# LJacksonPan/RaTrack

Hardware: AMD Instinct MI355X
Metric: radar frame-pairs/sec (backbone forward, eval) at B=64,N=256 per GPU (higher is better)
Workload: dtype f32 (2xfp16 split MFMA: three fp16 products per fp32 product, fp32 accumulate, power-of-two scales per matrix and position); 1 GPU; Track4D.backbone forward, B=64 frame-pairs x N=256 points per GPU, S=512 centroids, eval-mode BN, random-init weights, hipGraph=True, batches in flight=4; global_batch=64, parallelism=replicas x1 (no collective on the forward path)

## Files before the change

include/rtk_fused.h:

```cpp
#ifndef RTK_FUSED_H
#define RTK_FUSED_H

#include "rtk_pointnet2.h"

#ifdef __cplusplus
extern "C" {
#endif

#define RTK_MAX_SRC 4
#define RTK_MAX_LAYERS 4

typedef struct {
    const float *ptr;
    int pitch;
    int channels;
    int per_sample;
} rtk_src_t;

#define RTK_LAYER_SPLIT 0x100
typedef struct {
    const float *w_packed;
    const float *bias;
    int cin16, cout16;
    int act;
// ... 78 lines not shown
RTK_EXPORT int rtk_sa_scale_split(int samples, int n, int npoint, int nsample, const float *xyz, const float *new_xyz,
                                  const int *idx, const float *q, int q_pitch, int c1, const float *w1xyz_packed,
                                  const void *split_image, const float *image_scale, const float *bias2, float *out, int out_pitch,
                                  int out_offset, const int *src_nuniq, const int *dst_nuniq, rtk_stream_t stream);
RTK_EXPORT int rtk_sa_scale_split_serial(int samples, int n, int npoint, int nsample, const float *xyz, const float *new_xyz,
                                         const int *idx, const float *q, int q_pitch, int c1, const float *w1xyz_packed,
                                         const void *split_image, const float *image_scale, const float *bias2, float *out,
                                         int out_pitch, int out_offset, const int *src_nuniq, const int *dst_nuniq,
                                         rtk_stream_t stream);
RTK_EXPORT int rtk_split_mlp2(int positions, const float *x, const void *images, const float *image_scales, const float *bias1,
                              const float *bias2, float *y, rtk_stream_t stream);

RTK_EXPORT int rtk_prepare_inputs(int b, int n, const float *pc1, const float *pc2, const float *feature1,
                                  const float *feature2, float *xyz, float *raw, rtk_stream_t stream);

RTK_EXPORT int rtk_fps_centroids(int b, int n, int npoint, const float *xyz, int *idx, float *new_xyz, int *nuniq,
                                 int *tie, const int *n_valid, float *snap, int *first_tie, rtk_stream_t stream);

RTK_EXPORT int rtk_knn_point_masked(int b, int s, int n, int k, const float *query, const float *points, int64_t *idx,
                                    const int *n_valid, rtk_stream_t stream);

RTK_EXPORT int rtk_fps_relevel(int b, int npoint, int levels, const float *xyz1, const int *nuniq1, const int *tie,
                               int *idx, float *new_xyz, int *nuniq, int *tie_work, const int *idx1, const float *snap1,
                               int snap_pitch, const int *first_tie1, rtk_stream_t stream);

RTK_EXPORT int rtk_gru_step(int b, int layers, int hidden, const float *x, const float *h_in, const float *w_ih,
                            const float *w_hh, const float *b_ih, const float *b_hh, float *h_out, float *y,
                            rtk_stream_t stream);

RTK_EXPORT int rtk_gru_step_head(int b, int layers, int hidden, const float *x, const float *h_in, const float *w_ih,
                                 const float *w_hh, const float *b_ih, const float *b_hh, float *h_out, float *y, const float *head_wt,
                                 const float *head_bias, float *head_out, int head_cout, rtk_stream_t stream);

#define RTK_GT_MAX_JOBS 4
typedef struct {
    const float *wt, *bias;
    float *out;
    int cout, s0, count, out_pitch;
    const float *wt2;
    int s2;
} rtk_gterm_job_t;
RTK_EXPORT int rtk_global_terms(int samples, int cin, const float *g, int njobs, const rtk_gterm_job_t *jobs, float *bcast, int bcast_pitch,
                                int n, rtk_stream_t stream);

#define RTK_COPY_MAX_JOBS 8
typedef struct {
    const void *src;
    void *dst;
    long bytes;
} rtk_copy_job_t;
RTK_EXPORT int rtk_copy_multi(int njobs, const rtk_copy_job_t *jobs, rtk_stream_t stream);

RTK_EXPORT int rtk_to_channel_major(int samples, int n, int channels, const float *src, int src_pitch, int per_sample,
                                    float *dst, int dst_channels, int dst_channel_offset, rtk_stream_t stream);

RTK_EXPORT int rtk_ball_query_pair(int b, int n, int npoint, float radius1, int nsample1, float radius2, int nsample2,
                                   const float *new_xyz, const float *xyz, int *idx1, int *idx2, const int *nuniq,
                                   rtk_stream_t stream);

RTK_EXPORT int rtk_three_nn_masked(int b, int n, int m, const float *unknown, const float *known, float *dist2, int *idx,
                                   const int *unknown_nuniq, const int *known_nuniq, rtk_stream_t stream);

RTK_EXPORT int rtk_geometry_front(int b, int clouds, int n, int npoint, const float *frame1, const float *frame2, int channel_major,
                                  const float *feature1, const float *feature2, float *xyz, float *raw, int *fps_idx, float *new_xyz,
                                  int *nuniq, int *tie, int *first_tie, float *snap, const int *n_valid, int64_t *knn12, int64_t *knn11,
                                  const float *q1_w, float *q1_out, int q1_cout, rtk_stream_t stream);
// ... 72 lines not shown
```

ratrack_amd/abi.py:

```python
import ctypes

import torch

_i, _l, _f, _d, _p = ctypes.c_int, ctypes.c_long, ctypes.c_float, ctypes.c_double, ctypes.c_void_p
_ip, _fp, _pp, P = ctypes.POINTER(_i), ctypes.POINTER(_f), ctypes.POINTER(_p), ctypes.POINTER



class Src(ctypes.Structure):
    _fields_ = [("ptr", _p), ("pitch", _i), ("channels", _i), ("per_sample", _i)]


class Layer(ctypes.Structure):
    _fields_ = [("w_packed", _p), ("bias", _p), ("cin16", _i), ("cout16", _i), ("act", _i), ("inv_scale", _f)]


class Interp(ctypes.Structure):
    _fields_ = [("known_feats", _p), ("pitch", _i), ("channels", _i), ("m", _i), ("idx", _p), ("dist2", _p), ("nuniq", _p)]


class GtermJob(ctypes.Structure):
    _fields_ = [("wt", _p), ("bias", _p), ("out", _p), ("cout", _i), ("s0", _i), ("count", _i), ("out_pitch", _i), ("wt2", _p), ("s2", _i)]


# ... 121 lines not shown
    "rtk_group_points": [_i] * 5 + [_p] * 3 + [_p],
    "rtk_group_points_grad": [_i] * 5 + [_p] * 3 + [_p],
    "rtk_group_points_grad_set": [_i] * 5 + [_p] * 3 + [_p],
    "rtk_three_nn": [_i] * 3 + [_p] * 4 + [_p],
    "rtk_knn": [_i] * 4 + [_p] * 4 + [_p],
    "rtk_three_interpolate": [_i] * 4 + [_p] * 4 + [_p],
    "rtk_three_interpolate_grad": [_i] * 4 + [_p] * 4 + [_p],
    "rtk_three_interpolate_grad_set": [_i] * 4 + [_p] * 4 + [_p],
    "rtk_knn_point": [_i] * 4 + [_p] * 3 + [_p],
    "rtk_pointwise_mlp": [_i, _i, P(Interp), _i, P(Src), _p, _i, P(Layer), _p, _i, _i, _i, _p, _p, _p],
    "rtk_pointwise_mlp_pipelined": [_i, _i, P(Interp), _i, P(Src), _p, _i, P(Layer), _p, _i, _i, _i, _p, _p, _p],
    "rtk_pointwise_mlp_tap": [_i, _i, P(Interp), P(Layer), _p, _i, _p, P(Layer), _i, _p, _i, _p],
    "rtk_pointwise_mlp_tap_pipelined": [_i, _i, P(Interp), P(Layer), _p, _i, _p, P(Layer), _i, _p, _i, _p],
    "rtk_pointwise_mlp_pair": [_i, _i, _i, P(Src), _p, P(Layer), _p, _i, _i, _i, P(Layer), _p, _i, _p],
    "rtk_sa_scale": [_i] * 4 + [_p] * 4 + [_i, _i, _p, _i, P(Layer), _p, _i, _i, _p, _p, _p],
    "rtk_sa_scale_serial": [_i] * 4 + [_p] * 4 + [_i, _i, _p, _i, P(Layer), _p, _i, _i, _p, _p, _p],
    "rtk_cost_volume": [_i] * 3 + [_p] * 6 + [P(Layer), P(Layer), _p, _i, _p],
    "rtk_patch_cost": [_i] * 2 + [_p] * 3 + [_i, P(Layer), _p, _i, _i, _p],
    "rtk_patch_cost_wave16": [_i] * 2 + [_p] * 3 + [_i, P(Layer), _p, _i, _i, _p],
    "rtk_pack_split_layer": [_i, _i, _p, _i, _p, _p, _p],
    "rtk_cost_volume_split": [_i] * 3 + [_p] * 10 + [P(Layer), _p, _i, _p],
    "rtk_cost_volume_split_shared": [_i] * 3 + [_p] * 10 + [P(Layer), _p, _i, _i, _p],
    "rtk_cost_volume_split_gconst": [_i] * 3 + [_p] * 10 + [P(Layer), _p, _i, _i, _p],
    "rtk_cost_volume_split_term": [_i] * 3 + [_p] * 11 + [P(Layer), _p, _i, _i, _p],
    "rtk_sa_scale_split": [_i] * 4 + [_p] * 4 + [_i, _i, _p, _p, _p, _p, _p, _i, _i, _p, _p, _p],
    "rtk_sa_scale_split_serial": [_i] * 4 + [_p] * 4 + [_i, _i, _p, _p, _p, _p, _p, _i, _i, _p, _p, _p],
    "rtk_split_mlp2": [_i, _p, _p, _p, _p, _p, _p, _p],
    "rtk_prepare_inputs": [_i] * 2 + [_p] * 6 + [_p],
    "rtk_fps_centroids": [_i] * 3 + [_p] * 8 + [_p],
    "rtk_knn_point_masked": [_i] * 4 + [_p] * 4 + [_p],
    "rtk_fps_relevel": [_i] * 3 + [_p] * 9 + [_i, _p, _p],
    "rtk_gru_step": [_i] * 3 + [_p] * 8 + [_p],
    "rtk_gru_step_head": [_i] * 3 + [_p] * 11 + [_i, _p],
    "rtk_global_terms": [_i, _i, _p, _i, P(GtermJob), _p, _i, _i, _p],
    "rtk_copy_multi": [_i, P(CopyJob), _p],
    "rtk_to_channel_major": [_i] * 3 + [_p, _i, _i, _p, _i, _i, _p],
    "rtk_ball_query_pair": [_i] * 3 + [_f, _i, _f, _i] + [_p] * 5 + [_p],
    "rtk_three_nn_masked": [_i] * 3 + [_p] * 6 + [_p],
    "rtk_geometry_front": [_i] * 4 + [_p, _p, _i] + [_p] * 13 + [_p, _p, _i, _p],
    "rtk_geometry_tables": [_i] * 3 + [_p] * 3 + [_fp, _ip, _pp, _pp, _pp, _p],
    "rtk_to_channel_major_multi": [_i] * 3 + [_p, _p],
    "rtk_log_sinkhorn": [_i, _i, _p, _f, _i, _p, _p],
    "rtk_dbscan": [_i, _p, _i, _p, _p, _f, _d, _i, _p, _p],
    "rtk_dbscan_batched": [_p, _f, _d, _i, _i, _p, _p, _p, _p, _p, _l, _p],
    "rtk_object_descriptors": [_p, _i, _p, _p, _p, _p, _p, _p],
    "rtk_affinity_pairs": [_i, _i] + [_p] * 7 + [_p],
    "rtk_associate_batched": [_i] * 3 + [_p] * 7 + [_f, _i] + [_p] * 9 + [_p],
    "rtk_associate_optimal": [_i] * 3 + [_p] * 7 + [_d] + [_p] * 9 + [_p],
    "rtk_associate_optimal_lds_bytes": [_i],
    "rtk_track_memory": [_i] * 3 + [_p] * 21 + [_p],
    "rtk_track_memory_motion": [_i] * 3 + [_f] + [_p] * 24 + [_p],
    "rtk_track_max_objects": [],
    "rtk_gt_labels": [_p, _p, _p],
    "rtk_eval_frame": [_p, _p, _p, _p],
    "rtk_gt_objects_lds_bytes": [_i, _i],
    "rtk_track_score_lds_bytes": [_i, _i, _i],
    "rtk_track_score_memory_lds_bytes": [_i, _i, _i],
    "rtk_gt_objects": [_p, _p, _p],
    "rtk_track_score": [_p, _p, _p, _p],
    "rtk_track_score_logged": [_p, _p, _p, _p, _p],
    "rtk_track_score_memory": [_p, _p, _p, _p, _p, _p],
    "rtk_score_track_means": [_i, _p, _p, _p, _p],
    "rtk_score_thresholds": [_p, _p, _p, _i, _p, _p, _p],
    "rtk_score_replay": [_i, _i, _p, _p, _p, _p, _i, _p, _p, _p, _p],
    "rtk_score_hota": [_i, _i, _p, _p, _p, _i, _p, _p, _p, _p],
    "rtk_score_identity_lds_bytes": [_i],
# ... 69 lines not shown
```

ratrack_amd/csrc/fused_misc.hip:

```cpp
#include <math.h>

#include "assoc_common.h"
#include "rtk_common.h"
#include "rtk_fused.h"
#include "rtk_train.h"

__global__ void prepare_inputs_kernel(int b, int n, const float *__restrict__ pc1, const float *__restrict__ pc2,
                                      const float *__restrict__ f1, const float *__restrict__ f2, float *__restrict__ xyz,
                                      float *__restrict__ raw) {
    const long t = (long)blockIdx.x * blockDim.x + threadIdx.x;
    if (t >= 2L * b * n) return;
    const int s = (int)(t / n), p = (int)(t % n);
    const bool second = s >= b;
    const int sb = second ? s - b : s;
    const float *pc = second ? pc2 : pc1;
    const float *f = second ? f2 : f1;
    xyz[t * 3 + 0] = pc[((long)sb * 3 + 0) * n + p];
    xyz[t * 3 + 1] = pc[((long)sb * 3 + 1) * n + p];
    xyz[t * 3 + 2] = pc[((long)sb * 3 + 2) * n + p];
    *reinterpret_cast<float4 *>(raw + t * 4) = make_float4(f[((long)sb * 2 + 0) * n + p], f[((long)sb * 2 + 1) * n + p], 0.f, 0.f);
}

extern "C" int rtk_prepare_inputs(int b, int n, const float *pc1, const float *pc2, const float *feature1,
                                  const float *feature2, float *xyz, float *raw, rtk_stream_t stream) {
    RTK_REQUIRE(b > 0 && n > 0 && pc1 && pc2 && feature1 && feature2 && xyz && raw, "prepare_inputs: bad arguments");
    const long total = 2L * b * n;
    prepare_inputs_kernel<<<rtk_divup(total, 256), 256, 0, (hipStream_t)stream>>>(b, n, pc1, pc2, feature1, feature2, xyz, raw);
    RTK_CHECK_LAUNCH("prepare_inputs");
    return RTK_OK;
}

#define GRU_MAXL 8
constexpr int GRU_INFLIGHT = 32;
__global__ __launch_bounds__(384) void gru_step_kernel(int b, int layers, int hidden, const float *__restrict__ x,
                                                       const float *__restrict__ h_in, const float *__restrict__ w_ih,
                                                       const float *__restrict__ w_hh, const float *__restrict__ b_ih,
                                                       const float *__restrict__ b_hh, float *__restrict__ h_out,
                                                       float *__restrict__ y, const float *__restrict__ head_wt,
                                                       const float *__restrict__ head_bias, float *__restrict__ head_out, int head_cout) {
    __shared__ float s_x[128], s_h[128], s_gi[384], s_gh[384];
    const int s = blockIdx.x, t = threadIdx.x, H = hidden;
    if (t < H) s_x[t] = x[(long)s * H + t];
    for (int l = 0; l < layers; ++l) {
        if (t < H) s_h[t] = h_in[((long)l * b + s) * H + t];
        __syncthreads();
        if (t < 3 * H) {
            const float *wi = w_ih + (long)l * H * 3 * H + t;
            const float *wh = w_hh + (long)l * H * 3 * H + t;
            float ai = b_ih[l * 3 * H + t], ah = b_hh[l * 3 * H + t];
            for (int k0 = 0; k0 < H; k0 += GRU_INFLIGHT) {
                float wv[GRU_INFLIGHT], uv[GRU_INFLIGHT];
#pragma unroll
                for (int q = 0; q < GRU_INFLIGHT; ++q) {
                    wv[q] = wi[(long)(k0 + q) * 3 * H];
                    uv[q] = wh[(long)(k0 + q) * 3 * H];
                }
#pragma unroll
                for (int q = 0; q < GRU_INFLIGHT; ++q) {
                    ai = fmaf(wv[q], s_x[k0 + q], ai);
                    ah = fmaf(uv[q], s_h[k0 + q], ah);
                }
            }
            s_gi[t] = ai;
            s_gh[t] = ah;
        }
        __syncthreads();
        if (t < H) {
            const float r = 1.f / (1.f + expf(-(s_gi[t] + s_gh[t])));
            const float z = 1.f / (1.f + expf(-(s_gi[H + t] + s_gh[H + t])));
            const float nn = tanhf(s_gi[2 * H + t] + r * s_gh[2 * H + t]);
            const float hn = (1.f - z) * nn + z * s_h[t];
            h_out[((long)l * b + s) * H + t] = hn;
            s_x[t] = hn;
            if (l == layers - 1) y[(long)s * H + t] = hn;
        }
        __syncthreads();
    }
    if (head_wt) {
        for (int c = t; c < head_cout; c += blockDim.x) {
            float acc = head_bias ? head_bias[c] : 0.f;
            for (int k0 = 0; k0 < H; k0 += 16) {
                float wv[16];
#pragma unroll
                for (int q = 0; q < 16; ++q) wv[q] = head_wt[(long)(k0 + q) * head_cout + c];
#pragma unroll
                for (int q = 0; q < 16; ++q) acc = fmaf(wv[q], s_x[k0 + q], acc);
            }
            head_out[(long)s * head_cout + c] = acc;
        }
    }
}

extern "C" int rtk_gru_step(int b, int layers, int hidden, const float *x, const float *h_in, const float *w_ih,
                            const float *w_hh, const float *b_ih, const float *b_hh, float *h_out, float *y,
                            rtk_stream_t stream) {
    RTK_REQUIRE(b > 0 && layers > 0 && layers <= GRU_MAXL && hidden > 0 && hidden <= 128 && hidden % GRU_INFLIGHT == 0 && x && h_in && w_ih &&
                w_hh && b_ih && b_hh && h_out && y, "gru_step: bad arguments (hidden=%d, layers=%d)", hidden, layers);
    gru_step_kernel<<<b, 384, 0, (hipStream_t)stream>>>(b, layers, hidden, x, h_in, w_ih, w_hh, b_ih, b_hh, h_out, y, nullptr, nullptr, nullptr, 0);
    RTK_CHECK_LAUNCH("gru_step");
    return RTK_OK;
}

extern "C" int rtk_gru_step_head(int b, int layers, int hidden, const float *x, const float *h_in, const float *w_ih,
                                 const float *w_hh, const float *b_ih, const float *b_hh, float *h_out, float *y, const float *head_wt,
                                 const float *head_bias, float *head_out, int head_cout, rtk_stream_t stream) {
    RTK_REQUIRE(b > 0 && layers > 0 && layers <= GRU_MAXL && hidden > 0 && hidden <= 128 && hidden % GRU_INFLIGHT == 0 && x && h_in && w_ih &&
                w_hh && b_ih && b_hh && h_out && y && head_wt && head_out && head_cout > 0,
                "gru_step_head: bad arguments (hidden=%d, layers=%d, head_cout=%d)", hidden, layers, head_cout);
    gru_step_kernel<<<b, 384, 0, (hipStream_t)stream>>>(b, layers, hidden, x, h_in, w_ih, w_hh, b_ih, b_hh, h_out, y, head_wt, head_bias,
                                                        head_out, head_cout);
    RTK_CHECK_LAUNCH("gru_step_head");
    return RTK_OK;
}

struct GtParams {
    int samples, cin, njobs, n, bcast_pitch;
    const float *g;
    float *bcast;
    rtk_gterm_job_t job[RTK_GT_MAX_JOBS];
};

__global__ __launch_bounds__(256) void global_terms_kernel(const GtParams P) {
    __shared__ __attribute__((aligned(16))) float s_g[512];
    __shared__ float s_g2[RTK_GT_MAX_JOBS][512];
    const int s = blockIdx.x, t = threadIdx.x;
    for (int k = t; k < P.cin; k += 256) s_g[k] = P.g[(long)s * P.cin + k];
    for (int j = 0; j < P.njobs; ++j)
        if (P.job[j].wt2 && s >= P.job[j].s0 && s < P.job[j].s0 + P.job[j].count)
            for (int k = t; k < P.cin; k += 256) s_g2[j][k] = P.g[(long)(s - P.job[j].s0 + P.job[j].s2) * P.cin + k];
    __syncthreads();
    int total = 0;
    for (int j = 0; j < P.njobs; ++j)
        if (s >= P.job[j].s0 && s < P.job[j].s0 + P.job[j].count) total = (P.job[j].wt2 ? (total + 1) & ~1 : total) + (P.job[j].wt2 ? 2 : 1) * P.job[j].cout;
    for (int o = blockIdx.y * 256 + t; o < total; o += 256 * gridDim.y) {
        int c = -1, j = 0, base = 0;
        for (; j < P.njobs; ++j) {
            if (s < P.job[j].s0 || s >= P.job[j].s0 + P.job[j].count) continue;
            if (P.job[j].wt2) base = (base + 1) & ~1;
            const int span = (P.job[j].wt2 ? 2 : 1) * P.job[j].cout;
            if (o < base + span) { c = o - base; break; }
            base += span;
        }
        if (c < 0) continue;
        const rtk_gterm_job_t &J = P.job[j];
// ... 336 lines not shown
```

ratrack_amd/fused.py:

```python
import ctypes
import os
import types

import torch

from . import _lib
from . import pointnet2_hip as _native
from .abi import CopyJob as _CopyJob, GtermJob as _GtJob, Interp as _Interp, Layer as _Layer, Src as _Src, ptr as _ptr, stream as _stream

ACT_NONE, ACT_RELU, ACT_LEAKY, ACT_SIGMOID = 0, 1, 2, 3


def copy_multi(pairs):
    for i in range(0, len(pairs), 8):
        part = pairs[i:i + 8]
        jobs = (_CopyJob * len(part))()
        for j, (d, s_) in enumerate(part):
            assert d.is_contiguous() and s_.is_contiguous() and d.shape == s_.shape and d.dtype == s_.dtype and d.device == s_.device
            jobs[j].src, jobs[j].dst, jobs[j].bytes = s_.data_ptr(), d.data_ptr(), d.numel() * d.element_size()
        _lib.call("rtk_copy_multi", len(part), jobs, _stream())


def ceil16(c):
    return (c + 15) // 16 * 16
# ... 228 lines not shown
        _TRACE.append(("pointwise", rows, chain_a.macs))
    la, lb = chain_a.split_pair(chain_b)
    _lib.call("rtk_pointwise_mlp_pair", rows, rows_per_sample, len(srcs), _src_array(srcs), _ptr(sample_bias), la, *_colptr(out_a), chain_a.cout,
              chain_b.n, lb, out_b.data_ptr(), out_b_channels, _stream())
    return out_a, out_b


def offset_image(w4, device):
    cout = w4.shape[0]
    V = ceil16(cout) // 16
    wp = torch.zeros(V * 16, 4, dtype=torch.float32, device=device)
    wp[:cout] = w4.float().to(device)
    return wp.reshape(V, 16, 4).permute(0, 2, 1).contiguous().reshape(-1)


class _WeightNet:

    def __init__(self, sd, prefix, device):
        g = lambda k: sd[prefix + k].double()
        wa, ba = g(".mlp_convs.0.weight").reshape(8, 3), g(".mlp_convs.0.bias")
        wb, bb = g(".mlp_convs.1.weight").reshape(8, 8), g(".mlp_convs.1.bias")
        wc, bc = g(".mlp_convs.2.weight").reshape(-1, 8), g(".mlp_convs.2.bias")
        self.wa = offset_image(torch.cat([wa, ba[:, None]], 1), device)
        self.wb, self.bb = pack_layer(wb.to(device)), pad_bias(bb.to(device), 8)
        self.wc, self.bc = pack_layer(wc.to(device)), pad_bias(bc.to(device), wc.shape[0])
        arr = (_Layer * 3)()
        arr[0].w_packed, arr[0].cin16, arr[0].cout16 = self.wa.data_ptr(), 1, 1
        arr[1].w_packed, arr[1].bias, arr[1].cin16, arr[1].cout16 = self.wb.data_ptr(), self.bb.data_ptr(), 1, 1
        arr[2].w_packed, arr[2].bias, arr[2].cin16, arr[2].cout16 = self.wc.data_ptr(), self.bc.data_ptr(), 1, ceil16(wc.shape[0]) // 16
        self.arr = arr


SA_SPLIT = True


class _SAScale:

    def __init__(self, sd, prefix, nsample, radius, device):
        self.nsample, self.radius = nsample, float(radius)
        ws = []
        i = 0
        while (prefix + ".layer%d.conv.weight" % i) in sd:
            ws.append(fold_bn(sd[prefix + ".layer%d.conv.weight" % i], prefix + ".layer%d.bn.bn" % i, sd))
            i += 1
        w1, b1 = ws[0]
        self.c1 = w1.shape[0]
        self.wf = w1[:, 3:]
        self.w1img = offset_image(torch.cat([w1[:, :3], b1[:, None]], 1), device)
        self.chain = Chain([(w, b, ACT_RELU) for w, b in ws[1:]], device)
        self.cout = ws[-1][0].shape[0]
        self.split_image = None
        if SA_SPLIT and len(ws) == 2 and self.cout == 64 and self.c1 in (32, 64) and nsample in (16, 32) and torch.device(device).type == "cuda":
            w2 = ws[1][0].float().to(device).contiguous()
            self.split_bias = ws[1][1].float().to(device).contiguous()
            self.split_image, self.split_scale = pack_split_device(w2)
            torch.cuda.current_stream().synchronize()


class _PNHeadWeights:

    RADII = [[2, 4], [4, 8], [8, 16]]
    NSAMPLES = [[4, 8], [8, 16], [16, 32]]

    def __init__(self, sd, prefix, device):
        d = lambda k: sd[prefix + k].double()
        self.scales = [[_SAScale(sd, "%ssa%d.mlps.%d" % (prefix, l + 1, s), self.NSAMPLES[l][s], self.RADII[l][s], device)
# ... 283 lines not shown
    if not FOLD_LIN3:
        l3 = pointwise(S_ * S, S, [(sa3, 128, False)], W.lin3, new(S_ * S, 64), row_nuniq=nu[2])
    geo.wait("nn")
    d2, idx, m = geo.nn["fp3"]
    known, known_ch, chain = (sa3, 128, W.fp3c) if FOLD_LIN3 else (l3, 64, W.fp["fp3"])
    f3 = pointwise(S_ * S, S, [(t2[:, 0:64], 64, False)], chain, new(S_ * S, 128), row_nuniq=nu[1],
                   interp=(known, known_ch, m, idx.reshape(-1, 3), d2.reshape(-1, 3), nu[2]))
    d2, idx, m = geo.nn["fp2"]
    f2 = pointwise(S_ * S, S, [(t1[:, 0:32], 32, False)], W.fp["fp2"], new(S_ * S, 128), row_nuniq=nu[0],
                   interp=(f3, 128, m, idx.reshape(-1, 3), d2.reshape(-1, 3), nu[1]))
    d2, idx, m = geo.nn["fp1"]
    if gmax is None:
        gmax = torch.zeros(S_, 128, dtype=torch.float32, device=dev)
    out = out if out is not None else new(S_ * n, 128)
    interp = (f2, 128, m, idx.reshape(-1, 3), d2.reshape(-1, 3), nu[0])
    if tap is not None:
        pointwise_tap(S_ * n, n, W.fp["fp1"], out, gmax, interp, *tap)
    else:
        pointwise(S_ * n, n, [], W.fp["fp1"], out, interp=interp, colmax=gmax)
    return out, gmax


class FusedBackbone:

    def __init__(self, model, split=True):
        sd = {k: v.detach() for k, v in model.state_dict().items()}
        dev = next(model.parameters()).device
        self.dev = dev
        self.npoint = model.pn_head.sa1.npoint
        g = lambda k: torch.stack([sd["fd_layer.torchGRU.%s_l%d" % (k, l)].float() for l in range(5)])
        self.gru_wih = g("weight_ih").transpose(1, 2).contiguous()
        self.gru_whh = g("weight_hh").transpose(1, 2).contiguous()
        self.gru_bih, self.gru_bhh = g("bias_ih").contiguous(), g("bias_hh").contiguous()
        self.kernel_events = None
        self.kernel_token = None
        self._split_hook = None
        self.side, self.use_side_stream = None, True
        self.cv_shared = False
        self.proj_tap = True
        self.pair_readers = True
        self._last_cv = None
        self.enc = _PNHeadWeights(sd, "pn_head.", dev)
        self.dec = _PNHeadWeights(sd, "fd_layer.mse.", dev)
        z = lambda n: torch.zeros(n, dtype=torch.float64, device=sd["bin_score"].device)
        self.enc_q1 = Chain([(self.enc.wq1, z(32), ACT_NONE)], dev)
        self.enc_q1_w = self.enc.wq1.float().to(dev).contiguous()
        w0 = sd["fc_layer.mlp_convs.0.weight"].double().reshape(256, 515)
        b0 = sd["fc_layer.mlp_convs.0.bias"].double()
        self.p1_loc = Chain([(w0[:, 0:128], z(256), ACT_NONE)], dev)
        self.p2_loc = Chain([(w0[:, 256:384], z(256), ACT_NONE)], dev)
        tr = lambda w: w.float().t().contiguous().to(dev)
        self.p1_glob_wt, self.p1_glob_b = tr(w0[:, 128:256]), b0.float().to(dev).contiguous()
        self.p2_glob_wt = tr(w0[:, 384:512])
        self.cv_wd = offset_image(torch.cat([w0[:, 512:515], z(256)[:, None]], 1), dev)
        self.cv_layers = Chain([(sd["fc_layer.mlp_convs.%d.weight" % i].double().reshape(256, 256),
                                 sd["fc_layer.mlp_convs.%d.bias" % i].double(), ACT_LEAKY) for i in (1, 2)], dev)
        self.cv_split = bool(split)
        w23 = [sd["fc_layer.mlp_convs.%d.weight" % i].double().reshape(256, 256).float().to(dev).contiguous() for i in (1, 2)]
        self.cv_bias23 = torch.stack([sd["fc_layer.mlp_convs.%d.bias" % i].double().float() for i in (1, 2)]).to(dev).contiguous()
        self.cv_images = torch.empty(2 * SPLIT_IMAGE_256, dtype=torch.int16, device=dev)
        self.cv_scales = torch.empty(2, dtype=torch.float32, device=dev)
        for l, w in enumerate(w23):
            _lib.call("rtk_pack_split_layer", 256, 256, w.data_ptr(), 0, self.cv_images[l * SPLIT_IMAGE_256:].data_ptr(),
                      self.cv_scales[l:].data_ptr(), _stream())
        torch.cuda.current_stream().synchronize()
        self.wn1 = _WeightNet(sd, "fc_layer.weightnet1", dev)
        self.wn2 = _WeightNet(sd, "fc_layer.weightnet2", dev)
        def predictor(prefix, first_cols):
            layers = []
            for i in range(3):
                w, b = fold_bn(sd["%s.sf_mlp.%d.0.weight" % (prefix, i)], "%s.sf_mlp.%d.1" % (prefix, i), sd)
                layers.append([w, b, ACT_RELU])
            return layers
        cp = predictor("fd_layer.cp", None)
        wl, bl = sd["fd_layer.cp.linear.weight"].double(), sd["fd_layer.cp.linear.bias"].double()
        wc2 = sd["fd_layer.cp.conv2.weight"].double().reshape(3, 32)
        cp.append([wl @ wc2, bl, ACT_SIGMOID])
        self.cls_head = Chain([tuple(x) for x in cp], dev)
        fp = predictor("fd_layer.fp", None)
        w_first = fp[0][0]
        self.flow_glob_wt, self.flow_glob_b = tr(w_first[:, 128:256]), fp[0][1].float().to(dev).contiguous()
        fp[0] = [w_first[:, 0:128], z(128), ACT_RELU]
        fp.append([sd["fd_layer.fp.conv2.weight"].double().reshape(3, 32), z(3), ACT_NONE])
        self.flow_head = Chain([tuple(x) for x in fp], dev)
        wq = self.dec.wq1
        wq_pad = torch.zeros(32, 16, dtype=torch.float64, device=wq.device)
        wq_pad[:, :2] = wq[:, 0:2]
        self.dec_q1 = Chain([(torch.cat([wq_pad, wq[:, 2:130], wq[:, 258:514]], 1), z(32), ACT_NONE)], dev)
        self.dec_q1_glob_wt = tr(wq[:, 130:258])

    def backbone(self, pc1, pc2, feature1, feature2, h, n_valid=None):
        B, _, N = pc1.shape
        dev = pc1.device
        new = lambda rows, c: torch.empty(rows, c, dtype=torch.float32, device=dev)
        xyz = torch.empty(2 * B, N, 3, dtype=torch.float32, device=dev)
        raw = new(2 * B * N, 4)
        q1 = new(2 * B * N, 32)
        ins = [t.contiguous() for t in (pc1, pc2, feature1, feature2)]
        if self.side is None and self.use_side_stream:
            self.side = torch.cuda.Stream(device=dev)
        if n_valid is not None:
            n_valid = n_valid.to(device=dev, dtype=torch.int32).reshape(2 * B).contiguous()
        geo = Geometry(xyz, self.npoint, side=self.side if self.use_side_stream else None, knn_frames=B, n_valid=n_valid,
                       prepare=(ins[0], ins[1], ins[2], ins[3], raw), q1=(self.enc_q1_w, q1))
        geo.wait("front")
        if not geo.q1_done:
            pointwise(2 * B * N, N, [(raw, 2, False)], self.enc_q1, q1)
        elif _TRACE is not None:
            _TRACE.append(("pointwise", 2 * B * N, 64))
        feat12 = new(2 * B * N, 256)
        gmax = torch.zeros(3 * B, 128, dtype=torch.float32, device=dev)
        tap = self.proj_tap and self.cv_split and PW_SPLIT
        p12 = new(2 * B * N, 256) if tap else None
        loc, glob = run_pnhead(self.enc, geo, q1, out=feat12[:, 0:128], gmax=gmax[:2 * B],
                               tap=((self.p1_loc, self.p2_loc), B, p12) if tap else None)
        f1, f2 = loc[:B * N], loc[B * N:]
        sbq = new(B, 32)
        if tap:
            st = new(B, 256)
            global_terms(glob, [(self.p1_glob_wt, self.p1_glob_b, st, 0, self.p2_glob_wt, B), (self.dec_q1_glob_wt, None, sbq, 0)],
                         bcast=feat12[:, 128:], n=N)
            p1, p2 = p12[:B * N], p12[B * N:]
        else:
            st = None
            sb1, sb2 = new(B, 256), new(B, 256)
            global_terms(glob, [(self.p1_glob_wt, self.p1_glob_b, sb1, 0), (self.p2_glob_wt, None, sb2, B), (self.dec_q1_glob_wt, None, sbq, 0)],
                         bcast=feat12[:, 128:], n=N)
            p1 = pointwise(B * N, N, [(f1, 128, False)], self.p1_loc, new(B * N, 256), sample_bias=sb1)
            p2 = pointwise(B * N, N, [(f2, 128, False)], self.p2_loc, new(B * N, 256), sample_bias=sb2)
        x1, x2 = xyz[:B], xyz[B:]
        geo.wait("knn")
        knn1, knn2 = geo.knn
        cor1 = new(B * N, 256)
        self._last_cv = (B, N, x1, x2, knn1, p1, p2, cor1, st)
        if self._split_hook is not None:
            geo.events.clear()
            self._split_hook()
        else:
            ev = self.kernel_events
            if ev is not None:
                e0, e1 = torch.cuda.Event(enable_timing=True), torch.cuda.Event(enable_timing=True)
                e0.record()
            self._cost_volume(*self._last_cv)
            if ev is not None:
                e1.record()
                ev.append((e0, e1))
        cor = new(B * N, 256)
        if _TRACE is not None:
            _TRACE.append(("patch_cost", B * N * 16, (3 * 8 + 8 * 8 + 8 * 256) + 256))
        _lib.call("rtk_patch_cost", B, N, x1.data_ptr(), knn2.data_ptr(), cor1.data_ptr(), 256, self.wn2.arr, cor.data_ptr(), 256, 0,
                  _stream())
        cls = torch.empty(B, N, dtype=torch.float32, device=dev)
        dsrc = [(raw[:B * N], 2, False), (f1, 128, False), (cor, 256, False)]
        if self.pair_readers and PW_SPLIT:
            q1d, _ = pointwise_pair(B * N, N, dsrc, self.dec_q1, new(B * N, 32), sbq, self.cls_head, cls, 1)
        else:
            pointwise(B * N, N, [(cor, 256, False)], self.cls_head, cls, out_channels=1, channel_major=True)
            q1d = pointwise(B * N, N, dsrc, self.dec_q1, new(B * N, 32), sample_bias=sbq)
        prop, gfeat = run_pnhead(self.dec, geo.head(B), q1d, gmax=gmax[2 * B:])
        if h is None:
            h = torch.zeros(5, B, 128, device=dev, dtype=torch.float32)
        gout, h_out, sbf = self._gru_step(gfeat, h)
        flow = torch.empty(B, 3, N, dtype=torch.float32, device=dev)
        pointwise(B * N, N, [(prop, 128, False)], self.flow_head, flow, out_channels=3, sample_bias=sbf, channel_major=True)
        f12 = feat12.view(2 * B, N, 256).permute(0, 2, 1)
        pc1_features, pc2_features = f12[:B], f12[B:]
        cor_cm = cor.view(B, N, 256).permute(0, 2, 1)
        prop_cm = prop.view(B, N, 128).permute(0, 2, 1)
        return flow, h_out, cls, cor_cm, pc1_features, pc2_features, prop_cm

    def _cost_volume(self, B, N, x1, x2, knn1, p1, p2, cor1, sample_term=None):
        assert sample_term is None or self.cv_split
        if _TRACE is not None:
            _TRACE.append(("cost_volume", B * N * 16, 3 * 256 + 2 * 256 * 256 + (3 * 8 + 8 * 8 + 8 * 256) + 256))
        if self.cv_split:
            step = B if B * N <= CV_SPLIT_MAX_ROWS else max(1, CV_SPLIT_MAX_ROWS // N)
            for b0 in range(0, B, step):
                nb = min(step, B - b0)
                wgs = cv_shared_workgroups(nb, N, x1.device) if self.cv_shared else 0
                r0 = b0 * N
                if sample_term is not None:
                    _lib.call("rtk_cost_volume_split_term", nb, N, N, x1[b0:].data_ptr(), x2[b0:].data_ptr(), knn1[b0:].data_ptr(),
                              p1[r0:].data_ptr(), p2[r0:].data_ptr(), sample_term[b0:].data_ptr(), self.cv_wd.data_ptr(),
                              self.cv_images.data_ptr(), self.cv_scales.data_ptr(), self.cv_bias23[0].data_ptr(), self.cv_bias23[1].data_ptr(),
                              self.wn1.arr, cor1[r0:].data_ptr(), 256, wgs, _stream())
                    continue
                _lib.call("rtk_cost_volume_split_shared", nb, N, N, x1[b0:].data_ptr(), x2[b0:].data_ptr(), knn1[b0:].data_ptr(), p1[r0:].data_ptr(),
                          p2[r0:].data_ptr(), self.cv_wd.data_ptr(), self.cv_images.data_ptr(), self.cv_scales.data_ptr(),
                          self.cv_bias23[0].data_ptr(), self.cv_bias23[1].data_ptr(), self.wn1.arr, cor1[r0:].data_ptr(), 256, wgs, _stream())
            return
        _lib.call("rtk_cost_volume", B, N, N, x1.data_ptr(), x2.data_ptr(), knn1.data_ptr(), p1.data_ptr(), p2.data_ptr(),
                  self.cv_wd.data_ptr(), self.cv_layers.arr, self.wn1.arr, cor1.data_ptr(), 256, _stream())

    def _gru_step(self, x, h):
        L, B, H = h.shape
        if _TRACE is not None:
            _TRACE.append(("gru", B * L, 2 * 3 * H * H))
            _TRACE.append(("global_terms", B, H * self.flow_glob_wt.shape[1]))
        h_out = torch.empty_like(h)
        y = torch.empty(B, H, dtype=torch.float32, device=h.device)
        sbf = torch.empty(B, self.flow_glob_wt.shape[1], dtype=torch.float32, device=h.device)
        h = h.contiguous()
        _lib.call("rtk_gru_step_head", B, L, H, x.data_ptr(), h.data_ptr(), self.gru_wih.data_ptr(), self.gru_whh.data_ptr(),
                  self.gru_bih.data_ptr(), self.gru_bhh.data_ptr(), h_out.data_ptr(), y.data_ptr(), self.flow_glob_wt.data_ptr(),
                  self.flow_glob_b.data_ptr(), sbf.data_ptr(), sbf.shape[1], _stream())
        return y, h_out, sbf

    def clone(self):
        import copy
        e = copy.copy(self)
        e.side, e._last_cv, e.kernel_events, e.kernel_token = None, None, None, None
        return e

    def time_dominant_kernel(self, iters=20):
        assert self._last_cv is not None, "run backbone() first"
        ev = []
        for _ in range(iters):
            e0, e1 = torch.cuda.Event(enable_timing=True), torch.cuda.Event(enable_timing=True)
            e0.record()
            self._cost_volume(*self._last_cv)
            e1.record()
            ev.append((e0, e1))
        torch.cuda.synchronize()
        return ev

    def capture(self, pc1, pc2, feature1, feature2, h, split_cost_volume=False):
        static = [t.clone() for t in (pc1, pc2, feature1, feature2, h)]
        saved, self.kernel_events = self.kernel_events, None
        side = torch.cuda.Stream()
        side.wait_stream(torch.cuda.current_stream())
        with torch.cuda.stream(side):
            for _ in range(2):
                self.backbone(*static)
        torch.cuda.current_stream().wait_stream(side)
        if not split_cost_volume:
# ... 27 lines not shown
                outs = self.backbone(*static)
                g2.capture_end()
            finally:
                self._split_hook = None
        torch.cuda.current_stream().wait_stream(cap)
        cv_args = self._last_cv
        self.kernel_events = saved
        eng = self

        def step(*new_inputs):
            pairs = [(d, s_) for d, s_ in zip(static, new_inputs) if s_ is not None]
            if pairs:
                _copy_inputs(pairs)
            g1.replay()
            ev = eng.kernel_events
            if ev is not None:
                tok = eng.kernel_token
                if tok is not None and tok[0] is not None:
                    torch.cuda.current_stream().wait_event(tok[0])
                e0, e1 = torch.cuda.Event(enable_timing=True), torch.cuda.Event(enable_timing=True)
                e0.record()
            eng._cost_volume(*cv_args)
            if ev is not None:
                e1.record()
                ev.append((e0, e1))
                if tok is not None:
                    tok[0] = e1
            g2.replay()
            return outs
        step.graph = (g1, g2)
        return step


def global_terms(g, jobs, bcast=None, n=0):
    samples, cin = g.shape
    arr = (_GtJob * max(len(jobs), 1))()
    for j, job in enumerate(jobs):
        wt, bias, out, s0 = job[:4]
        wt2, s2 = job[4:] if len(job) > 4 else (None, 0)
        assert wt.shape == (cin, out.shape[1]) and out.is_contiguous() and wt.is_contiguous()
        assert wt2 is None or (wt2.shape == wt.shape and wt2.is_contiguous())
        arr[j].wt, arr[j].bias, arr[j].out = wt.data_ptr(), bias.data_ptr() if bias is not None else None, out.data_ptr()
        arr[j].cout, arr[j].s0, arr[j].count, arr[j].out_pitch = out.shape[1], s0, out.shape[0], out.shape[1]
        arr[j].wt2, arr[j].s2 = wt2.data_ptr() if wt2 is not None else None, s2
    if _TRACE is not None:
        _TRACE.append(("global_terms", 1, sum(cin * j[2].shape[0] * j[2].shape[1] * (2 if len(j) > 4 else 1) for j in jobs)))
    bptr, bpitch = _colptr(bcast) if bcast is not None else (None, 0)
    _lib.call("rtk_global_terms", samples, cin, g.data_ptr(), len(jobs), arr, bptr, bpitch, n, _stream())


def _copy_inputs(pairs):
    if all(d.is_contiguous() and s_.is_contiguous() and d.shape == s_.shape and d.dtype == s_.dtype and d.device == s_.device and
           d.element_size() == 4 for d, s_ in pairs):
        copy_multi(pairs)
    else:
        torch._foreach_copy_([p[0] for p in pairs], [p[1] for p in pairs])


class GraphPipeline:

    def __init__(self, model_or_engine, example_inputs, depth=2, split_cost_volume=False):
        eng = model_or_engine if isinstance(model_or_engine, FusedBackbone) else FusedBackbone(model_or_engine)
        if depth > 2:
            eng = eng.clone()
            eng.use_side_stream = False
            eng.cv_shared = True
# ... 32 lines not shown
```

Measured before the change: 122,600 frame-pairs/s.

## Split GRU hidden-state matmul into an early kernel off the critical path

```diff
diff --git a/include/rtk_fused.h b/include/rtk_fused.h
--- a/include/rtk_fused.h
+++ b/include/rtk_fused.h
@@ -134,6 +134,12 @@
                                  const float *w_hh, const float *b_ih, const float *b_hh, float *h_out, float *y, const float *head_wt,
                                  const float *head_bias, float *head_out, int head_cout, rtk_stream_t stream);
 
+RTK_EXPORT int rtk_gru_hidden_terms(int b, int layers, int hidden, const float *h_in, const float *w_hh, const float *b_hh, float *gh,
+                                    rtk_stream_t stream);
+RTK_EXPORT int rtk_gru_chain_head(int b, int layers, int hidden, const float *x, const float *h_in, const float *w_ih4, const float *b_ih,
+                                  const float *gh, float *h_out, float *y, const float *head_wt, const float *head_bias, float *head_out,
+                                  int head_cout, rtk_stream_t stream);
+
 #define RTK_GT_MAX_JOBS 4
 typedef struct {
     const float *wt, *bias;
diff --git a/ratrack_amd/abi.py b/ratrack_amd/abi.py
--- a/ratrack_amd/abi.py
+++ b/ratrack_amd/abi.py
@@ -177,6 +177,8 @@
     "rtk_fps_relevel": [_i] * 3 + [_p] * 9 + [_i, _p, _p],
     "rtk_gru_step": [_i] * 3 + [_p] * 8 + [_p],
     "rtk_gru_step_head": [_i] * 3 + [_p] * 11 + [_i, _p],
+    "rtk_gru_hidden_terms": [_i] * 3 + [_p] * 4 + [_p],
+    "rtk_gru_chain_head": [_i] * 3 + [_p] * 10 + [_i, _p],
     "rtk_global_terms": [_i, _i, _p, _i, P(GtermJob), _p, _i, _i, _p],
     "rtk_copy_multi": [_i, P(CopyJob), _p],
     "rtk_to_channel_major": [_i] * 3 + [_p, _i, _i, _p, _i, _i, _p],
diff --git a/ratrack_amd/csrc/fused_misc.hip b/ratrack_amd/csrc/fused_misc.hip
--- a/ratrack_amd/csrc/fused_misc.hip
+++ b/ratrack_amd/csrc/fused_misc.hip
@@ -32,6 +32,15 @@
 
 #define GRU_MAXL 8
 constexpr int GRU_INFLIGHT = 32;
+
+__device__ __forceinline__ float gru_gates(float gi_r, float gh_r, float gi_z, float gh_z, float gi_n, float gh_n, float h) {
+    const float r = 1.f / (1.f + expf(-(gi_r + gh_r)));
+    const float z = 1.f / (1.f + expf(-(gi_z + gh_z)));
+    const float nn = tanhf(gi_n + r * gh_n);
+    const float hn = (1.f - z) * nn + z * h;
+    return hn;
+}
+
 __global__ __launch_bounds__(384) void gru_step_kernel(int b, int layers, int hidden, const float *__restrict__ x,
                                                        const float *__restrict__ h_in, const float *__restrict__ w_ih,
                                                        const float *__restrict__ w_hh, const float *__restrict__ b_ih,
@@ -66,10 +75,7 @@
         }
         __syncthreads();
         if (t < H) {
-            const float r = 1.f / (1.f + expf(-(s_gi[t] + s_gh[t])));
-            const float z = 1.f / (1.f + expf(-(s_gi[H + t] + s_gh[H + t])));
-            const float nn = tanhf(s_gi[2 * H + t] + r * s_gh[2 * H + t]);
-            const float hn = (1.f - z) * nn + z * s_h[t];
+            const float hn = gru_gates(s_gi[t], s_gh[t], s_gi[H + t], s_gh[H + t], s_gi[2 * H + t], s_gh[2 * H + t], s_h[t]);
             h_out[((long)l * b + s) * H + t] = hn;
             s_x[t] = hn;
             if (l == layers - 1) y[(long)s * H + t] = hn;
@@ -110,6 +116,218 @@
     gru_step_kernel<<<b, 384, 0, (hipStream_t)stream>>>(b, layers, hidden, x, h_in, w_ih, w_hh, b_ih, b_hh, h_out, y, head_wt, head_bias,
                                                         head_out, head_cout);
     RTK_CHECK_LAUNCH("gru_step_head");
+    return RTK_OK;
+}
+
+#ifndef GRU_TILE
+#define GRU_TILE 2
+#endif
+static_assert(GRU_TILE >= 1 && GRU_TILE <= 8, "GRU_TILE");
+
+template <int NS>
+__device__ __forceinline__ void gru_hidden_tile(int b, int l, int s0, int H, const float *__restrict__ h_in, const float *__restrict__ w_hh,
+                                                const float *__restrict__ b_hh, float *__restrict__ gh, float (*s_h)[128]) {
+    const int t = threadIdx.x;
+    const float *hl = h_in + ((long)l * b + s0) * H;
+    for (int e = t; e < NS * H; e += blockDim.x) s_h[e / H][e % H] = hl[e];
+    __syncthreads();
+    if (t >= 3 * H) return;
+    const float *wh = w_hh + (long)l * H * 3 * H + t;
+    float ah[NS];
+    const float bias = b_hh[l * 3 * H + t];
+#pragma unroll
+    for (int s = 0; s < NS; ++s) ah[s] = bias;
+    for (int k0 = 0; k0 < H; k0 += GRU_INFLIGHT) {
+        float uv[GRU_INFLIGHT];
+#pragma unroll
+        for (int q = 0; q < GRU_INFLIGHT; ++q) uv[q] = wh[(long)(k0 + q) * 3 * H];
+#pragma unroll
+        for (int q = 0; q < GRU_INFLIGHT; ++q)
+#pragma unroll
+            for (int s = 0; s < NS; ++s) ah[s] = fmaf(uv[q], s_h[s][k0 + q], ah[s]);
+    }
+#pragma unroll
+    for (int s = 0; s < NS; ++s) gh[((long)l * b + s0 + s) * 3 * H + t] = ah[s];
+}
+
+template <int NS>
+__device__ __forceinline__ void gru_hidden_dispatch(int ns, int b, int l, int s0, int H, const float *__restrict__ h_in,
+                                                    const float *__restrict__ w_hh, const float *__restrict__ b_hh, float *__restrict__ gh,
+                                                    float (*s_h)[128]) {
+    if (ns == NS) gru_hidden_tile<NS>(b, l, s0, H, h_in, w_hh, b_hh, gh, s_h);
+    else if constexpr (NS > 1) gru_hidden_dispatch<NS - 1>(ns, b, l, s0, H, h_in, w_hh, b_hh, gh, s_h);
+}
+
+__global__ __launch_bounds__(384) void gru_hidden_terms_kernel(int b, int hidden, const float *__restrict__ h_in, const float *__restrict__ w_hh,
+                                                               const float *__restrict__ b_hh, float *__restrict__ gh) {
+    __shared__ float s_h[GRU_TILE][128];
+    const int s0 = blockIdx.x * GRU_TILE;
+    gru_hidden_dispatch<GRU_TILE>(min(GRU_TILE, b - s0), b, blockIdx.y, s0, hidden, h_in, w_hh, b_hh, gh, s_h);
+}
+
+extern "C" int rtk_gru_hidden_terms(int b, int layers, int hidden, const float *h_in, const float *w_hh, const float *b_hh, float *gh,
+                                    rtk_stream_t stream) {
+    RTK_REQUIRE(b > 0 && layers > 0 && layers <= GRU_MAXL && hidden > 0 && hidden <= 128 && hidden % GRU_INFLIGHT == 0 && h_in && w_hh && b_hh &&
+                gh, "gru_hidden_terms: bad arguments (hidden=%d, layers=%d)", hidden, layers);
+    gru_hidden_terms_kernel<<<dim3(rtk_divup(b, GRU_TILE), layers), 384, 0, (hipStream_t)stream>>>(b, hidden, h_in, w_hh, b_hh, gh);
+    RTK_CHECK_LAUNCH("gru_hidden_terms");
+    return RTK_OK;
+}
+
+template <int NS, int QS>
+__device__ __forceinline__ void gru_sum_set(float (&ai)[NS], const float4 (&w)[QS / 4], const float (*s_x)[128], int k0) {
+    constexpr int KC = NS > 4 ? 4 : 8;
+    static_assert(QS % KC == 0, "QS");
+#pragma unroll
+    for (int q0 = 0; q0 < QS; q0 += KC) {
+#pragma unroll
+        for (int q = q0; q < q0 + KC; q += 4)
+#pragma unroll
+            for (int s = 0; s < NS; ++s) {
+                ai[s] = fmaf(w[q / 4].x, s_x[s][k0 + q], ai[s]);
+                ai[s] = fmaf(w[q / 4].y, s_x[s][k0 + q + 1], ai[s]);
+                ai[s] = fmaf(w[q / 4].z, s_x[s][k0 + q + 2], ai[s]);
+                ai[s] = fmaf(w[q / 4].w, s_x[s][k0 + q + 3], ai[s]);
+            }
+#pragma unroll
+        for (int s = 0; s < NS; ++s) asm volatile("" : "+v"(ai[s]) : : "memory");
+    }
+}
+
+template <int NS, int QS>
+__device__ __forceinline__ void gru_chain_tile(int b, int layers, int s0, const float *__restrict__ x, const float *__restrict__ h_in,
+                                               const float4 *__restrict__ w_ih4, const float *__restrict__ b_ih, const float *__restrict__ gh,
+                                               float *__restrict__ h_out, float *__restrict__ y, const float *__restrict__ head_wt,
+                                               const float *__restrict__ head_bias, float *__restrict__ head_out, int head_cout,
+                                               float (*s_x)[128], float (*s_gi)[384], float (*s_ho)[GRU_TILE][128]) {
+    constexpr int H = 4 * QS;
+    constexpr int UNITS = NS * H;
+    constexpr int PASSES = (UNITS + 383) / 384;
+    const int t = threadIdx.x;
+    const bool row = 3 * H == 384 || t < 3 * H;
+    for (int e = t; e < UNITS; e += 384) s_x[e / H][e % H] = x[(long)s0 * H + e];
+    const unsigned col = t;
+    float bias = 0.f;
+    float4 w0[QS / 4], w1[QS / 4], w2[QS / 4], w3[QS / 4];
+#define GRU_REQUEST(w_, layer_, part_)                                                                                                           \
+    _Pragma("unroll") for (int q = 0; q < QS / 4; ++q) w_[q] = (w_ih4 + ((layer_) * QS + (part_) * (QS / 4) + q) * 3 * H)[col];
+    if (row) {
+        bias = b_ih[t];
+        GRU_REQUEST(w0, 0, 0)
+        GRU_REQUEST(w1, 0, 1)
+        GRU_REQUEST(w2, 0, 2)
+        GRU_REQUEST(w3, 0, 3)
+    }
+    __syncthreads();
+    for (int l = 0; l < layers; ++l) {
+        const int ln = min(l + 1, layers - 1);
+        float bias_next = 0.f;
+        if (row) bias_next = b_ih[ln * 3 * H + t];
+        float g_r[PASSES], g_z[PASSES], g_n[PASSES], g_h[PASSES];
+#pragma unroll
+        for (int p = 0; p < PASSES; ++p) {
+            const int e = min(t + p * 384, UNITS - 1), s = e / H, j = e % H;
+            const float *g = gh + ((long)l * b + s0 + s) * 3 * H + j;
+            g_r[p] = g[0];
+            g_z[p] = g[H];
+            g_n[p] = g[2 * H];
+            g_h[p] = h_in[((long)l * b + s0 + s) * H + j];
+        }
+        if (row) {
+            float ai[NS];
+#pragma unroll
+            for (int s = 0; s < NS; ++s) ai[s] = bias;
+            gru_sum_set<NS, QS>(ai, w0, s_x, 0);
+            GRU_REQUEST(w0, ln, 0)
+            gru_sum_set<NS, QS>(ai, w1, s_x, QS);
+            GRU_REQUEST(w1, ln, 1)
+            gru_sum_set<NS, QS>(ai, w2, s_x, 2 * QS);
+            GRU_REQUEST(w2, ln, 2)
+            gru_sum_set<NS, QS>(ai, w3, s_x, 3 * QS);
+            GRU_REQUEST(w3, ln, 3)
+#pragma unroll
+            for (int s = 0; s < NS; ++s) s_gi[s][t] = ai[s];
+        }
+        bias = bias_next;
+        __syncthreads();
+#pragma unroll
+        for (int p = 0; p < PASSES; ++p) {
+            const int e = min(t + p * 384, UNITS - 1), s = e / H, j = e % H;
+            const float hn = gru_gates(s_gi[s][j], g_r[p], s_gi[s][H + j], g_z[p], s_gi[s][2 * H + j], g_n[p], g_h[p]);
+            if (t + p * 384 < UNITS) {
+                s_ho[l][s][j] = hn;
+                s_x[s][j] = hn;
+            }
+        }
+        __syncthreads();
+    }
+#undef GRU_REQUEST
+    for (int c = t; c < head_cout; c += 384) {
+        float acc[NS];
+        const float bias = head_bias ? head_bias[c] : 0.f;
+#pragma unroll
+        for (int s = 0; s < NS; ++s) acc[s] = bias;
+        for (int k0 = 0; k0 < H; k0 += 16) {
+            float wv[16];
+#pragma unroll
+            for (int q = 0; q < 16; ++q) wv[q] = head_wt[(long)(k0 + q) * head_cout + c];
+#pragma unroll
+            for (int q = 0; q < 16; ++q)
+#pragma unroll
+                for (int s = 0; s < NS; ++s) acc[s] = fmaf(wv[q], s_x[s][k0 + q], acc[s]);
+#pragma unroll
+            for (int s = 0; s < NS; ++s) asm volatile("" : "+v"(acc[s]) : : "memory");
+        }
+#pragma unroll
+        for (int s = 0; s < NS; ++s) head_out[(long)(s0 + s) * head_cout + c] = acc[s];
+    }
+    for (int l = 0; l < layers; ++l)
+        for (int e = t; e < UNITS; e += 384) h_out[((long)l * b + s0) * H + e] = s_ho[l][e / H][e % H];
+    for (int e = t; e < UNITS; e += 384) y[(long)s0 * H + e] = s_x[e / H][e % H];
+}
+
+template <int NS, int QS>
+__device__ __forceinline__ void gru_chain_dispatch(int ns, int b, int layers, int s0, const float *__restrict__ x, const float *__restrict__ h_in,
+                                                   const float4 *__restrict__ w_ih4, const float *__restrict__ b_ih, const float *__restrict__ gh,
+                                                   float *__restrict__ h_out, float *__restrict__ y, const float *__restrict__ head_wt,
+                                                   const float *__restrict__ head_bias, float *__restrict__ head_out, int head_cout,
+                                                   float (*s_x)[128], float (*s_gi)[384], float (*s_ho)[GRU_TILE][128]) {
+    if (ns == NS) gru_chain_tile<NS, QS>(b, layers, s0, x, h_in, w_ih4, b_ih, gh, h_out, y, head_wt, head_bias, head_out, head_cout, s_x, s_gi, s_ho);
+    else if constexpr (NS > 1)
+        gru_chain_dispatch<NS - 1, QS>(ns, b, layers, s0, x, h_in, w_ih4, b_ih, gh, h_out, y, head_wt, head_bias, head_out, head_cout, s_x, s_gi, s_ho);
+}
+
+__global__ __launch_bounds__(384) void gru_chain_head_kernel(int b, int layers, int hidden, const float *__restrict__ x,
+                                                             const float *__restrict__ h_in, const float4 *__restrict__ w_ih4,
+                                                             const float *__restrict__ b_ih, const float *__restrict__ gh,
+                                                             float *__restrict__ h_out, float *__restrict__ y,
+                                                             const float *__restrict__ head_wt, const float *__restrict__ head_bias,
+                                                             float *__restrict__ head_out, int head_cout) {
+    __shared__ float s_x[GRU_TILE][128], s_gi[GRU_TILE][384], s_ho[GRU_MAXL][GRU_TILE][128];
+    const int s0 = blockIdx.x * GRU_TILE, ns = min(GRU_TILE, b - s0);
+#define GRU_CHAIN_CASE(QS_)                                                                                                                      \
+    case 4 * QS_:                                                                                                                                \
+        gru_chain_dispatch<GRU_TILE, QS_>(ns, b, layers, s0, x, h_in, w_ih4, b_ih, gh, h_out, y, head_wt, head_bias, head_out, head_cout, s_x,    \
+                                          s_gi, s_ho);                                                                                                \
+        break;
+    switch (hidden) {
+        GRU_CHAIN_CASE(32)
+        GRU_CHAIN_CASE(24)
+        GRU_CHAIN_CASE(16)
+        GRU_CHAIN_CASE(8)
+    }
+#undef GRU_CHAIN_CASE
+}
+
+extern "C" int rtk_gru_chain_head(int b, int layers, int hidden, const float *x, const float *h_in, const float *w_ih4, const float *b_ih,
+                                  const float *gh, float *h_out, float *y, const float *head_wt, const float *head_bias, float *head_out,
+                                  int head_cout, rtk_stream_t stream) {
+    RTK_REQUIRE(b > 0 && layers > 0 && layers <= GRU_MAXL && hidden > 0 && hidden <= 128 && hidden % GRU_INFLIGHT == 0 && x && h_in && w_ih4 &&
+                ((uintptr_t)w_ih4 & 15) == 0 && b_ih && gh && h_out && y && head_wt && head_out && head_cout > 0,
+                "gru_chain_head: bad arguments (hidden=%d, layers=%d, head_cout=%d)", hidden, layers, head_cout);
+    gru_chain_head_kernel<<<rtk_divup(b, GRU_TILE), 384, 0, (hipStream_t)stream>>>(b, layers, hidden, x, h_in, reinterpret_cast<const float4 *>(w_ih4), b_ih, gh, h_out,
+                                                                                  y, head_wt,                                                                                   head_bias, head_out, head_cout);
+    RTK_CHECK_LAUNCH("gru_chain_head");
     return RTK_OK;
 }
 
diff --git a/ratrack_amd/fused.py b/ratrack_amd/fused.py
--- a/ratrack_amd/fused.py
+++ b/ratrack_amd/fused.py
@@ -284,6 +284,7 @@
 
 
 SA_SPLIT = True
+GRU_SPLIT = True
 
 
 class _SAScale:
@@ -633,6 +634,7 @@
         self.gru_wih = g("weight_ih").transpose(1, 2).contiguous()
         self.gru_whh = g("weight_hh").transpose(1, 2).contiguous()
         self.gru_bih, self.gru_bhh = g("bias_ih").contiguous(), g("bias_hh").contiguous()
+        self.gru_wih4 = gru_quads(self.gru_wih)
         self.kernel_events = None
         self.kernel_token = None
         self._split_hook = None
@@ -698,6 +700,10 @@
         raw = new(2 * B * N, 4)
         q1 = new(2 * B * N, 32)
         ins = [t.contiguous() for t in (pc1, pc2, feature1, feature2)]
+        if h is None:
+            h = torch.zeros(5, B, 128, device=dev, dtype=torch.float32)
+        h = h.contiguous()
+        gh = self._gru_hidden_terms(h) if GRU_SPLIT else None
         if self.side is None and self.use_side_stream:
             self.side = torch.cuda.Stream(device=dev)
         if n_valid is not None:
@@ -759,9 +765,7 @@
             pointwise(B * N, N, [(cor, 256, False)], self.cls_head, cls, out_channels=1, channel_major=True)
             q1d = pointwise(B * N, N, dsrc, self.dec_q1, new(B * N, 32), sample_bias=sbq)
         prop, gfeat = run_pnhead(self.dec, geo.head(B), q1d, gmax=gmax[2 * B:])
-        if h is None:
-            h = torch.zeros(5, B, 128, device=dev, dtype=torch.float32)
-        gout, h_out, sbf = self._gru_step(gfeat, h)
+        gout, h_out, sbf = self._gru_step(gfeat, h, gh)
         flow = torch.empty(B, 3, N, dtype=torch.float32, device=dev)
         pointwise(B * N, N, [(prop, 128, False)], self.flow_head, flow, out_channels=3, sample_bias=sbf, channel_major=True)
         f12 = feat12.view(2 * B, N, 256).permute(0, 2, 1)
@@ -793,7 +797,13 @@
         _lib.call("rtk_cost_volume", B, N, N, x1.data_ptr(), x2.data_ptr(), knn1.data_ptr(), p1.data_ptr(), p2.data_ptr(),
                   self.cv_wd.data_ptr(), self.cv_layers.arr, self.wn1.arr, cor1.data_ptr(), 256, _stream())
 
-    def _gru_step(self, x, h):
+    def _gru_hidden_terms(self, h):
+        L, B, H = h.shape
+        gh = torch.empty(L, B, 3 * H, dtype=torch.float32, device=h.device)
+        _lib.call("rtk_gru_hidden_terms", B, L, H, h.data_ptr(), self.gru_whh.data_ptr(), self.gru_bhh.data_ptr(), gh.data_ptr(), _stream())
+        return gh
+
+    def _gru_step(self, x, h, gh=None):
         L, B, H = h.shape
         if _TRACE is not None:
             _TRACE.append(("gru", B * L, 2 * 3 * H * H))
@@ -802,6 +812,11 @@
         y = torch.empty(B, H, dtype=torch.float32, device=h.device)
         sbf = torch.empty(B, self.flow_glob_wt.shape[1], dtype=torch.float32, device=h.device)
         h = h.contiguous()
+        if gh is not None:
+            _lib.call("rtk_gru_chain_head", B, L, H, x.data_ptr(), h.data_ptr(), self.gru_wih4.data_ptr(), self.gru_bih.data_ptr(),
+                      gh.data_ptr(), h_out.data_ptr(), y.data_ptr(), self.flow_glob_wt.data_ptr(), self.flow_glob_b.data_ptr(),
+                      sbf.data_ptr(), sbf.shape[1], _stream())
+            return y, h_out, sbf
         _lib.call("rtk_gru_step_head", B, L, H, x.data_ptr(), h.data_ptr(), self.gru_wih.data_ptr(), self.gru_whh.data_ptr(),
                   self.gru_bih.data_ptr(), self.gru_bhh.data_ptr(), h_out.data_ptr(), y.data_ptr(), self.flow_glob_wt.data_ptr(),
                   self.flow_glob_b.data_ptr(), sbf.data_ptr(), sbf.shape[1], _stream())
@@ -895,6 +910,11 @@
         return step
 
 
+def gru_quads(w_t):
+    L, H, G = w_t.shape
+    return w_t.reshape(L, H // 4, 4, G).permute(0, 1, 3, 2).contiguous()
+
+
 def global_terms(g, jobs, bcast=None, n=0):
     samples, cin = g.shape
     arr = (_GtJob * max(len(jobs), 1))()
```

Result: no change. 122,700 frame-pairs/s (median of 2 runs) (+0.1%).
